# sunshanlu/ORB_SLAM2_ROS2

Hardware: AMD Instinct MI355X
Metric: stereo frames/sec (extract+match) KITTI-00 1241x376; HBM GB/s vs roofline (higher is better)
Workload: dtype u8; 1 GPU; Single 1241x376 KITTI-shaped stereo pair, 8-level pyramid, 2000 FAST+rBRIEF keypoints per image, searchByStereo; batched (512 pairs per step, 512 of them distinct synthetic frames).  `value` is DEVICE-RESIDENT; the checks, rooflines, host_io, sequence job, content sweep, CPU baseline and extra legs run with --full; io=device-resident, n_features=2000, levels=8

## Files before the change

orb_slam2_ros2_amd/csrc/k_brief.hip:

```cpp
#include <hip/hip_runtime.h>
#include <cstdio>
#include <cstring>

#include "orb_math.h"
#include "orbfe_internal.h"
#ifdef BRIEF_STAMPS
namespace orbfe { extern __device__ unsigned long long g_rt_t[4][8]; }
#define RT_STAMP(k) { __syncthreads(); if (tid == 0 && blockIdx.y == 0) orbfe::g_rt_t[k][0] = __builtin_amdgcn_s_memrealtime(); }
#define RTP_STAMP(k) { __syncthreads(); if (tid == 0 && blockIdx.y == 0) orbfe::g_rt_t[k][r] = __builtin_amdgcn_s_memrealtime(); }
#endif
#include "rowtable_body.h"
#include "wave_ops.h"

namespace orbfe {

typedef unsigned long long UmaxPacked;

template <int CTRL, int ROW_MASK>
__device__ __forceinline__ int dpp_i32(int v) {
  return __builtin_amdgcn_update_dpp(0, v, CTRL, ROW_MASK, 0xf, false);
}
__device__ __forceinline__ int wave_sum_i(int v) {
  v += dpp_i32<0x111, 0xf>(v);
  v += dpp_i32<0x112, 0xf>(v);
  v += dpp_i32<0x114, 0xf>(v);
  v += dpp_i32<0x118, 0xf>(v);
  v += dpp_i32<0x142, 0xa>(v);
  v += dpp_i32<0x143, 0xc>(v);
  return __builtin_amdgcn_readlane(v, 63);
}

__device__ __forceinline__ int locate_level(const int32_t* __restrict__ sc, int n_levels, int k, int* j_out, int* total_out) {
  int level = -1, acc = 0, j = 0;
  for (int l = 0; l < n_levels; ++l) {
    const int c = sc[l];
    if (level < 0 && k < acc + c) {
      level = l;
      j = k - acc;
    }
    acc += c;
  }
  *j_out = j;
  *total_out = acc;
  return level;
}

__global__ __launch_bounds__(256) void k_kplist(const LevelDev* __restrict__ lv, int n_levels, const uint32_t* __restrict__ sel,
                                                const int32_t* __restrict__ sel_count, int n_features, uint4* __restrict__ kpl) {
  const int k = blockIdx.x * 256 + threadIdx.x;
  const int img = blockIdx.y;
  if (k >= n_features) return;
  int j, total;
  const int level = locate_level(sel_count + (size_t)img * n_levels, n_levels, k, &j, &total);
  uint4 e = make_uint4(0xFFFFu, 0u, 0u, 0u);
  if (level >= 0) {
    const LevelDev& L = lv[level];
    const uint32_t rec = sel[(size_t)img * n_features + L.quota_off + j];
    e.x = (ORBFE_REC_X(rec) + ORBFE_EDGE) | ((ORBFE_REC_Y(rec) + ORBFE_EDGE) << 16);
    e.y = (uint32_t)level | (ORBFE_REC_R(rec) << 8);
    e.z = L.plane_off;
    e.w = (uint32_t)L.stride;
  }
  kpl[(size_t)img * n_features + k] = e;
}

__global__ __launch_bounds__(256) void k_ic_moments(const uint8_t* __restrict__ pyr, size_t img_pitch, const uint4* __restrict__ kpl,
                                                    int n_features, UmaxPacked umax, int2* __restrict__ moments) {
  __shared__ uint32_t s_mask[256];
  {
    const int it = threadIdx.x >> 4, sb = threadIdx.x & 15;
    const int dy = (sb >> 3) + 2 * it - 15;
    const int ady = dy < 0 ? -dy : dy;
    uint32_t mask = 0u;
    if (ady <= 15) {
      const int d = (int)((umax >> (4 * ady)) & 15ull);
      const int dx0 = 4 * (sb & 7) - 15;
      const int lo = max(0, -d - dx0), hi = min(3, d - dx0);
      mask = (hi >= lo) ? ((0xFFFFFFFFu >> (8 * (3 - hi))) & (0xFFFFFFFFu << (8 * lo))) : 0u;
    }
    s_mask[threadIdx.x] = mask;
  }
  __syncthreads();
  const int lane = threadIdx.x & 63, sub = lane & 15;
  const int k = (blockIdx.x * 4 + (threadIdx.x >> 6)) * 4 + (lane >> 4);
  const int img = blockIdx.y;
  const bool in_range = k < n_features;
  const uint4 e = in_range ? kpl[(size_t)img * n_features + k] : make_uint4(0xFFFFu, 0u, 0u, 0u);
  const bool valid = (e.x & 0xFFFFu) != 0xFFFFu;
  const int x = valid ? (int)(e.x & 0xFFFFu) : 16, y = valid ? (int)(e.x >> 16) : 16;
  const uint8_t* I = pyr + (size_t)img * img_pitch;
  const uint32_t plane = valid ? e.z : 0u;
  const int stride = valid ? (int)e.w : 64;
  constexpr int NIT = 16;
  const uint32_t a0 = plane + (uint32_t)mad24u(y - 15 + (sub >> 3), stride, x - 15 + 4 * (sub & 7));
  const uint32_t step = 2u * (uint32_t)stride;
  uint32_t wv[NIT];
#pragma unroll
  for (int it = 0; it < NIT; ++it) {
    uint32_t w;
    __builtin_memcpy(&w, I + (a0 + (uint32_t)it * step), 4);
    wv[it] = w;
  }
  uint32_t S = 0u, Wp = 0u, T = 0u;
#pragma unroll
  for (int it = 0; it < NIT; ++it) {
    const uint32_t w = wv[it] & s_mask[it * 16 + sub];
    S = __builtin_amdgcn_udot4(w, 0x01010101u, S, false);
    Wp = __builtin_amdgcn_udot4(w, 0x03020100u, Wp, false);
    T = __builtin_amdgcn_udot4(w, 0x01010101u * (uint32_t)it, T, false);
  }
  const int S18 = (int)(S & 0x3FFFFu);
  int m10 = (4 * (sub & 7) - 15) * S18 + (int)Wp;
  int m01 = ((sub >> 3) - 15) * S18 + 2 * (int)T;
#pragma unroll
  for (int sh = 0; sh < 4; ++sh) {
    m10 += (sh == 0) ? dpp_i32<0x111, 0xf>(m10) : (sh == 1) ? dpp_i32<0x112, 0xf>(m10) : (sh == 2) ? dpp_i32<0x114, 0xf>(m10) : dpp_i32<0x118, 0xf>(m10);
    m01 += (sh == 0) ? dpp_i32<0x111, 0xf>(m01) : (sh == 1) ? dpp_i32<0x112, 0xf>(m01) : (sh == 2) ? dpp_i32<0x114, 0xf>(m01) : dpp_i32<0x118, 0xf>(m01);
  }
  if (sub == 15 && valid) moments[(size_t)img * n_features + k] = make_int2(m10, m01);
}

__device__ __forceinline__ KpX kpx_of(const orbfe_keypoint& kp, float sf) {
#pragma clang fp contract(off)
  const float fxq = kp.x / sf, fyq = kp.y / sf;
  int qx = (int)fxq, qy = (int)fyq;
  qx -= (qx > fxq);
  qy -= (qy > fyq);
  KpX r;
  r.x = kp.x;
  r.q = ORBFE_KPX_Q(kp.octave, qx, qy);
  return r;
}

__global__ __launch_bounds__(256) void k_orient(const LevelDev* __restrict__ lv, const uint4* __restrict__ kpl, int n_features,
                                                const int2* __restrict__ moments, double2* __restrict__ sincos,
                                                orbfe_keypoint* __restrict__ kps, KpAux* __restrict__ aux, KpX* __restrict__ kx,
                                                double* __restrict__ theta_out, int rows0, const int32_t* __restrict__ sel_count, int n_levels,
                                                int32_t* __restrict__ n_kp, orbfe_keypoint* __restrict__ kps_host, int32_t* __restrict__ n_kp_host) {
#pragma clang fp contract(off)
  const int k = blockIdx.x * 256 + threadIdx.x;
  const int img = blockIdx.y;
  if (k == 0) {
    int total = 0;
    for (int l = 0; l < n_levels; ++l) total += sel_count[(size_t)img * n_levels + l];
    n_kp[img] = total;
    if (n_kp_host) n_kp_host[img] = total;
  }
  const uint4 e = (k < n_features) ? kpl[(size_t)img * n_features + k] : make_uint4(0xFFFFu, 0u, 0u, 0u);
  if ((e.x & 0xFFFFu) != 0xFFFFu) {
    const int level = (int)(e.y & 0xFFu);
    const LevelDev& L = lv[level];
    const int x = (int)(e.x & 0xFFFFu), y = (int)(e.x >> 16);
    const size_t o = (size_t)img * n_features + k;
    const int2 m = moments[o];
    const double theta = orbmath::det_atan2((double)m.y, (double)m.x);
    double sn, cs;
    orbmath::det_sincos(theta, &sn, &cs);
    sincos[o] = make_double2(sn, cs);
    orbfe_keypoint kp;
    kp.x = (float)x * L.sf;
    kp.y = (float)y * L.sf;
    kp.size = 7.0f;
    kp.angle = (float)(theta / 3.14159265358979323846 * 180);
    kp.response = (float)((e.y >> 8) & 0xFFu);
    kp.octave = level;
    kp.class_id = -1;
    kps[o] = kp;
  #ifndef EXP_NO_KPS_HOST
  if (kps_host) kps_host[o] = kp;
#endif
    kx[o] = kpx_of(kp, L.sf);
    const float r = (float)(2.0 * (double)L.sf);
    const unsigned row = (unsigned)__float2int_rn(kp.y);
    KpAux a;
    a.row_max = (int16_t)min(rows0, __float2int_rn((float)row + r + 1.0f));
    a.row_min = (int16_t)max(0, __float2int_rn((float)row - r));
    aux[o] = a;
    if (theta_out) theta_out[o] = theta;
  }
}

template <bool WITH_ORIENT>
__global__ __launch_bounds__(256) void k_list_moments_orient(const LevelDev* __restrict__ lv, int n_levels, const uint32_t* __restrict__ sel,
                                                             const int32_t* __restrict__ sel_count, int n_features,
                                                             const uint8_t* __restrict__ pyr, size_t img_pitch, UmaxPacked umax,
                                                             uint4* __restrict__ kpl, int2* __restrict__ moments, double2* __restrict__ sincos,
                                                             orbfe_keypoint* __restrict__ kps, KpAux* __restrict__ aux, KpX* __restrict__ kx,
                                                             double* __restrict__ theta_out, int rows0, int32_t* __restrict__ n_kp,
                                                             orbfe_keypoint* __restrict__ kps_host, int32_t* __restrict__ n_kp_host,
                                                             int32_t* __restrict__ rt_flags) {
#pragma clang fp contract(off)
  __shared__ uint32_t s_mask[256];
  if (rt_flags && blockIdx.x == 0 && threadIdx.x < 8) rt_flags[blockIdx.y * 8 + threadIdx.x] = 0;
  {
    const int it = threadIdx.x >> 4, sb = threadIdx.x & 15;
    const int dy = (sb >> 3) + 2 * it - 15;
    const int ady = dy < 0 ? -dy : dy;
    uint32_t mask = 0u;
    if (ady <= 15) {
      const int d = (int)((umax >> (4 * ady)) & 15ull);
      const int dx0 = 4 * (sb & 7) - 15;
      const int lo = max(0, -d - dx0), hi = min(3, d - dx0);
      mask = (hi >= lo) ? ((0xFFFFFFFFu >> (8 * (3 - hi))) & (0xFFFFFFFFu << (8 * lo))) : 0u;
    }
    s_mask[threadIdx.x] = mask;
  }
  __syncthreads();
  const int lane = threadIdx.x & 63, sub = lane & 15;
  const int k = (blockIdx.x * 4 + (threadIdx.x >> 6)) * 4 + (lane >> 4);
  const int img = blockIdx.y;
  const bool in_range = k < n_features;
  uint4 e = make_uint4(0xFFFFu, 0u, 0u, 0u);
  int level = -1, total = 0;
  {
    int j;
    level = locate_level(sel_count + (size_t)img * n_levels, n_levels, in_range ? k : 0x7FFFFFFF, &j, &total);
    if (level >= 0) {
      const LevelDev& L = lv[level];
      const uint32_t rec = sel[(size_t)img * n_features + L.quota_off + j];
      e.x = (ORBFE_REC_X(rec) + ORBFE_EDGE) | ((ORBFE_REC_Y(rec) + ORBFE_EDGE) << 16);
      e.y = (uint32_t)level | (ORBFE_REC_R(rec) << 8);
      e.z = L.plane_off;
      e.w = (uint32_t)L.stride;
    }
  }
  if (WITH_ORIENT && k == 0 && sub == 15) {
    n_kp[img] = total;
    if (n_kp_host) n_kp_host[img] = total;
  }
  const bool valid = (e.x & 0xFFFFu) != 0xFFFFu;
  const int x = valid ? (int)(e.x & 0xFFFFu) : 16, y = valid ? (int)(e.x >> 16) : 16;
  const uint8_t* I = pyr + (size_t)img * img_pitch;
  const uint32_t plane = valid ? e.z : 0u;
  const int stride = valid ? (int)e.w : 64;
  constexpr int NIT = 16;
  const uint32_t a0 = plane + (uint32_t)mad24u(y - 15 + (sub >> 3), stride, x - 15 + 4 * (sub & 7));
  const uint32_t step = 2u * (uint32_t)stride;
  uint32_t wv[NIT];
#pragma unroll
  for (int it = 0; it < NIT; ++it) {
    uint32_t w;
    __builtin_memcpy(&w, I + (a0 + (uint32_t)it * step), 4);
    wv[it] = w;
  }
  uint32_t S = 0u, Wp = 0u, T = 0u;
#pragma unroll
  for (int it = 0; it < NIT; ++it) {
    const uint32_t w = wv[it] & s_mask[it * 16 + sub];
    S = __builtin_amdgcn_udot4(w, 0x01010101u, S, false);
    Wp = __builtin_amdgcn_udot4(w, 0x03020100u, Wp, false);
    T = __builtin_amdgcn_udot4(w, 0x01010101u * (uint32_t)it, T, false);
  }
  const int S18 = (int)(S & 0x3FFFFu);
  int m10 = (4 * (sub & 7) - 15) * S18 + (int)Wp;
  int m01 = ((sub >> 3) - 15) * S18 + 2 * (int)T;
#pragma unroll
  for (int sh = 0; sh < 4; ++sh) {
    m10 += (sh == 0) ? dpp_i32<0x111, 0xf>(m10) : (sh == 1) ? dpp_i32<0x112, 0xf>(m10) : (sh == 2) ? dpp_i32<0x114, 0xf>(m10) : dpp_i32<0x118, 0xf>(m10);
    m01 += (sh == 0) ? dpp_i32<0x111, 0xf>(m01) : (sh == 1) ? dpp_i32<0x112, 0xf>(m01) : (sh == 2) ? dpp_i32<0x114, 0xf>(m01) : dpp_i32<0x118, 0xf>(m01);
  }
  if (sub != 15 || !in_range) return;
  const size_t o = (size_t)img * n_features + k;
  kpl[o] = e;
  if (!valid) return;
  moments[o] = make_int2(m10, m01);
  if (!WITH_ORIENT) return;
  const LevelDev& L = lv[level];
  const double theta = orbmath::det_atan2((double)m01, (double)m10);
  double sn, cs;
  orbmath::det_sincos(theta, &sn, &cs);
  sincos[o] = make_double2(sn, cs);
  orbfe_keypoint kp;
  kp.x = (float)x * L.sf;
  kp.y = (float)y * L.sf;
  kp.size = 7.0f;
  kp.angle = (float)(theta / 3.14159265358979323846 * 180);
  kp.response = (float)((e.y >> 8) & 0xFFu);
  kp.octave = level;
  kp.class_id = -1;
  kps[o] = kp;
#ifndef EXP_NO_KPS_HOST
  if (kps_host) kps_host[o] = kp;
#endif
  kx[o] = kpx_of(kp, L.sf);
  const float r = (float)(2.0 * (double)L.sf);
  const unsigned row = (unsigned)__float2int_rn(kp.y);
  KpAux a;
  a.row_max = (int16_t)min(rows0, __float2int_rn((float)row + r + 1.0f));
  a.row_min = (int16_t)max(0, __float2int_rn((float)row - r));
  aux[o] = a;
  if (theta_out) theta_out[o] = theta;
}

#define BRIEF_R 18
#define BRIEF_ROWS (2 * BRIEF_R + 1)
#define BRIEF_PITCH 48
#define BRIEF_WIN_BYTES 2048

#ifndef BRIEF_WAVES
#define BRIEF_WAVES 4
#endif
#ifndef BRIEF_KPW
#define BRIEF_KPW 2
#endif
#ifdef BRIEF_STAMPS
__device__ unsigned long long g_rt_t[4][8];
__device__ unsigned long long g_bs_rec[8192][6];
#define BS_DECL const unsigned bs_w = ((blockIdx.y * 520u + blockIdx.x) * BRIEF_WAVES + (threadIdx.x >> 6)) & 8191u; const unsigned long long bs_t0 = __builtin_amdgcn_s_memrealtime(); unsigned long long bs_t1 = 0, bs_ta = 0, bs_tb = 0;
#define BS_MID if (!bs_t1) bs_t1 = __builtin_amdgcn_s_memrealtime();
#define BS_END(kind) if ((threadIdx.x & 63) == 0) { asm volatile("s_waitcnt vmcnt(0) lgkmcnt(0)" ::: "memory"); g_bs_rec[bs_w][0] = bs_t0, g_bs_rec[bs_w][1] = bs_t1, g_bs_rec[bs_w][2] = __builtin_amdgcn_s_memrealtime(), g_bs_rec[bs_w][3] = kind, g_bs_rec[bs_w][4] = bs_ta, g_bs_rec[bs_w][5] = bs_tb; }
#else
#define BS_DECL
#define BS_MID
#define BS_END(kind)
#endif
struct BriefRowTable {
  const KpAux* aux;
  const int32_t* n_kp;
  uint32_t* rowoff;
  uint16_t* rowlist;
  int32_t* n_match;
  int rows, list_cap, slot0, n_brief_blocks;
  int stage_cap;
  int32_t* flags;
};
__global__ __launch_bounds__(64 * BRIEF_WAVES) __attribute__((amdgpu_waves_per_eu(8, 8))) void k_brief(const uint8_t* __restrict__ blur, size_t img_pitch,
                                              const uint4* __restrict__ kpl, int n_features, const int8_t* __restrict__ pattern,
                                              const double2* __restrict__ sincos, uint8_t* __restrict__ desc, uint8_t* __restrict__ desc_host,
                                              BriefRowTable rt) {
#pragma clang fp contract(off)
  struct __attribute__((aligned(16))) Lds {
    double rc[BRIEF_WAVES][40];
    uint8_t win[BRIEF_WAVES][2][BRIEF_WIN_BYTES];
    double rs[BRIEF_WAVES][40];
  };
  static_assert(BRIEF_ROWS * BRIEF_PITCH <= BRIEF_WIN_BYTES && BRIEF_WIN_BYTES == 2 * 64 * 16 && BRIEF_PITCH % 16 == 0, "a window is two 16-byte LDS-DMA instructions");
  static_assert((sizeof(double) * 40 * BRIEF_WAVES) % 16 == 0, "the LDS-DMA destination is 16-byte aligned");
  static_assert(sizeof(double) * 40 * BRIEF_WAVES + 2 * BRIEF_WIN_BYTES * BRIEF_WAVES > 255 * 8 &&
                    (sizeof(double) * 40 * BRIEF_WAVES + 2 * BRIEF_WIN_BYTES * BRIEF_WAVES) % 512 != 0,
                "rc[w] and rs[w] must not be reachable by one ds_read2(st64)_b64");
  __shared__ Lds lds;
  BS_DECL
  if (rt.rowoff && (int)blockIdx.x >= rt.n_brief_blocks) {
    static_assert(sizeof(Lds) >= 9000, "the table's row counters borrow the descriptor kernel's LDS (launch_orient_brief checks the row count against 9000 bytes)");
    uint32_t* cnt = (uint32_t*)&lds;
    const int slot = rt.slot0 + (int)blockIdx.y;
    const int r = (int)blockIdx.x - rt.n_brief_blocks;
    if (rt.flags) {
      if (r == 0 && threadIdx.x == 0) rt.n_match[slot >> 1] = 0;
      const int rpw = (rt.rows + 7) >> 3;
      extern __shared__ __attribute__((aligned(16))) uint2 brief_bands[];
      rowtable_build_part(rt.aux + (size_t)blockIdx.y * n_features, min(rt.n_kp[blockIdx.y], n_features), rt.rows, rt.list_cap,
                          rt.rowoff + (size_t)slot * (rt.rows + 1), rt.rowlist + (size_t)slot * rt.list_cap, cnt, cnt + rpw + 12, (int)threadIdx.x, r,
                          rt.flags + (size_t)blockIdx.y * 8, rt.stage_cap > 0 ? brief_bands : nullptr, rt.stage_cap / 4);
      BS_END(2)
      return;
    }
    if (r != 0) return;
    if (threadIdx.x == 0) rt.n_match[slot >> 1] = 0;
    extern __shared__ __attribute__((aligned(16))) uint16_t brief_stage[];
    rowtable_build(rt.aux + (size_t)blockIdx.y * n_features, min(rt.n_kp[blockIdx.y], n_features), rt.rows, rt.list_cap,
                   rt.rowoff + (size_t)slot * (rt.rows + 1), rt.rowlist + (size_t)slot * rt.list_cap, cnt, cnt + rt.rows, (int)threadIdx.x,
                   rt.stage_cap > 0 ? brief_stage : nullptr, rt.stage_cap);
    BS_END(2)
    return;
  }
  const int lane = threadIdx.x & 63;
  const int wave = __builtin_amdgcn_readfirstlane((int)(threadIdx.x >> 6));
  double* rc = lds.rc[wave];
  double* rs = lds.rs[wave];
  const int per_xcd = rt.n_brief_blocks >> 3;
  const int kb = ((int)blockIdx.x & 7) * per_xcd + ((int)blockIdx.x >> 3);
  const int k0 = (kb * BRIEF_WAVES + wave) * BRIEF_KPW;
  const int img = blockIdx.y;
  if (k0 >= n_features) return;
  const uint4* list = kpl + (size_t)img * n_features;
  const double2* sc = sincos + (size_t)img * n_features;
  const uint8_t* W = blur + (size_t)img * img_pitch;
  const int k_last = min(k0 + BRIEF_KPW, n_features) - 1;
  uint32_t tp0 = *(const uint32_t*)(pattern + (0 * 64 + lane) * 4), tp1 = *(const uint32_t*)(pattern + (1 * 64 + lane) * 4);
  uint32_t tp2 = *(const uint32_t*)(pattern + (2 * 64 + lane) * 4), tp3 = *(const uint32_t*)(pattern + (3 * 64 + lane) * 4);
#ifdef BRIEF_STAMPS
  asm volatile("s_waitcnt vmcnt(0)" :: "v"(tp0), "v"(tp1), "v"(tp2), "v"(tp3) : "memory");
  bs_t1 = __builtin_amdgcn_s_memrealtime();
#endif
  const int u1 = min(lane + 64, BRIEF_ROWS * (BRIEF_PITCH / 16) - 1);
  const uint32_t row_a = (uint32_t)lane / 3u, row_b = (uint32_t)u1 / 3u;
  const uint32_t col_a = 16u * ((uint32_t)lane - 3u * row_a), col_b = 16u * ((uint32_t)u1 - 3u * row_b);
  typedef __attribute__((address_space(3))) uint8_t* lds_dst_t;
  typedef const __attribute__((address_space(1))) uint8_t* glb_src_t;
  auto request = [&](const uint4 e, int b) __attribute__((always_inline)) {
    const bool used = (e.x & 0xFFFFu) != 0xFFFFu;
    const int x = used ? (int)(e.x & 0xFFFFu) : BRIEF_R, y = used ? (int)(e.x >> 16) : BRIEF_R;
    const uint32_t plane = used ? e.z : 0u;
    const uint32_t stride = used ? e.w : 0u;
    const uint32_t xa = (uint32_t)(x - BRIEF_R) & ~3u;
    const uint32_t s0 = plane + (uint32_t)(y - BRIEF_R) * stride + xa;
    uint8_t* dst = lds.win[wave][b];
    __builtin_amdgcn_global_load_lds((glb_src_t)(W + (s0 + col_a + __umul24(row_a, stride))), (lds_dst_t)dst, 16, 0, 0);
    __builtin_amdgcn_global_load_lds((glb_src_t)(W + (s0 + col_b + __umul24(row_b, stride))), (lds_dst_t)(dst + 1024), 16, 0, 0);
  };
  uint4 e_cur = list[k0];
  uint4 e_nxt = list[min(k0 + 1, k_last)];
  double2 sc_cur = sc[k0];
#ifdef BRIEF_STAMPS
  asm volatile("s_waitcnt lgkmcnt(0)" ::: "memory");
  bs_ta = __builtin_amdgcn_s_memrealtime();
#endif
  asm volatile("" : "+v"(tp0), "+v"(tp1), "+v"(tp2), "+v"(tp3));
  request(e_cur, 0);
#ifdef BRIEF_STAMPS
  asm volatile("s_waitcnt vmcnt(0)" ::: "memory");
  bs_tb = __builtin_amdgcn_s_memrealtime();
#endif
#pragma unroll
  for (int i = 0; i < BRIEF_KPW; ++i) {
    const int k = k0 + i;
    if (k > k_last) break;
    uint4 e_nn = e_nxt;
    double2 sc_nxt = sc_cur;
    if (i + 2 < BRIEF_KPW) e_nn = list[min(k + 2, k_last)];
    if (i + 1 < BRIEF_KPW && k < k_last) {
      request(e_nxt, (i + 1) & 1);
      sc_nxt = sc[k + 1];
      asm volatile("s_waitcnt vmcnt(2)" ::: "memory");
    } else {
      asm volatile("s_waitcnt vmcnt(0)" ::: "memory");
    }
    __builtin_amdgcn_wave_barrier();
    if ((e_cur.x & 0xFFFFu) != 0xFFFFu) {
      const int x = (int)(e_cur.x & 0xFFFFu), y = (int)(e_cur.x >> 16);
      const int xa = (x - BRIEF_R) & ~3;
      const uint8_t* win = lds.win[wave][i & 1];
      const double sn = sc_cur.x, cs = sc_cur.y;
      if (lane <= 2 * BRIEF_R) {
        const double v = (double)(float)(lane - BRIEF_R);
        rc[lane] = v * cs;
        rs[lane] = v * sn;
      }
      __builtin_amdgcn_fence(__ATOMIC_RELEASE, "wavefront");
      __builtin_amdgcn_wave_barrier();
      BS_MID
      const float px = (float)x, py = (float)y;
      typedef const __attribute__((address_space(3))) uint8_t* lds_bytes_t;
      auto magic_row = [](int y0w) { return (float)(12582912 - (y0w & ~1)); };
      auto magic_col = [](int xa, int y0w, int pitch, int lds_addr) { return (float)(12582912 - xa + lds_addr - (y0w & 1) * pitch); };
      const int y0w = y - BRIEF_R;
      const float magic_y = magic_row(y0w);
      const float magic_x = magic_col(xa, y0w, BRIEF_PITCH, (int)(uint32_t)(uintptr_t)(lds_bytes_t)win);
      auto tests = [&](const uint32_t tpg) __attribute__((always_inline)) -> unsigned long long {
        const int x1 = (int)(int8_t)(tpg & 255u), y1 = (int)(int8_t)((tpg >> 8) & 255u);
        const int x2 = (int)(int8_t)((tpg >> 16) & 255u), y2 = (int)(int8_t)(tpg >> 24);
        const float p1x = (float)(rc[x1 + BRIEF_R] - rs[y1 + BRIEF_R]);
        const float p1y = (float)(rs[x1 + BRIEF_R] + rc[y1 + BRIEF_R]);
        const float p2x = (float)(rc[x2 + BRIEF_R] - rs[y2 + BRIEF_R]);
        const float p2y = (float)(rs[x2 + BRIEF_R] + rc[y2 + BRIEF_R]);
        const uint32_t a1 = (uint32_t)mad24u(__float_as_int((py + p1y) + magic_y), BRIEF_PITCH, __float_as_int((px + p1x) + magic_x)) & 0xFFFFu;
        const uint32_t a2 = (uint32_t)mad24u(__float_as_int((py + p2y) + magic_y), BRIEF_PITCH, __float_as_int((px + p2x) + magic_x)) & 0xFFFFu;
        const int v1 = *(lds_bytes_t)(uintptr_t)a1;
        const int v2 = *(lds_bytes_t)(uintptr_t)a2;
        return __ballot(v1 < v2);
      };
      const unsigned long long bits0 = tests(tp0), bits1 = tests(tp1), bits2 = tests(tp2), bits3 = tests(tp3);
      if (lane < 4) {
        unsigned long long* d64 = (unsigned long long*)(desc + ((size_t)img * n_features + k) * 32);
        unsigned long long b = bits0;
        if (lane == 1) b = bits1;
        if (lane == 2) b = bits2;
        if (lane == 3) b = bits3;
        d64[lane] = b;
        if (desc_host) ((unsigned long long*)(desc_host + ((size_t)img * n_features + k) * 32))[lane] = b;
      }
      __builtin_amdgcn_fence(__ATOMIC_RELEASE, "wavefront");
      __builtin_amdgcn_wave_barrier();
    }
    if (i + 1 < BRIEF_KPW) {
      e_cur = e_nxt;
      e_nxt = e_nn;
      sc_cur = sc_nxt;
    }
  }
  BS_END(1)
}
#ifdef BRIEF_STAMPS
}
extern "C" void orbfe_debug_brief_stamps() {
  static unsigned long long rec[8192][6];
  (void)hipDeviceSynchronize();
  (void)hipMemcpyFromSymbol(rec, HIP_SYMBOL(orbfe::g_bs_rec), sizeof(rec));
  unsigned long long first = ~0ull, last = 0, n = 0, sum = 0, mx = 0, mid = 0, rt0 = 0, rt1 = 0, dlast = 0, sa = 0, sb = 0, ma = 0, mb = 0, smax = 0;
  for (int w = 0; w < 8192; ++w) {
    if (!rec[w][3]) continue;
    first = first < rec[w][0] ? first : rec[w][0], last = last > rec[w][2] ? last : rec[w][2];
    if (rec[w][3] == 1) {
      ++n, sum += rec[w][2] - rec[w][0], mx = mx > rec[w][2] - rec[w][0] ? mx : rec[w][2] - rec[w][0], mid += rec[w][1] ? rec[w][1] - rec[w][0] : 0;
      dlast = dlast > rec[w][2] ? dlast : rec[w][2];
      sa += rec[w][4] - rec[w][0], sb += rec[w][5] - rec[w][4];
      ma = ma > rec[w][4] - rec[w][0] ? ma : rec[w][4] - rec[w][0], mb = mb > rec[w][5] - rec[w][4] ? mb : rec[w][5] - rec[w][4];
    }
  }
  printf("BRIEF stamps (last launch): %llu descriptor waves, launch span %.2f us, last descriptor wave ends at %.2f us; wave mean %.2f max %.2f us, pattern words arrive after %.2f us (mean)\n",
         n, (last - first) * 0.01, (dlast - first) * 0.01, n ? sum * 0.01 / n : 0.0, mx * 0.01, n ? mid * 0.01 / n : 0.0);
  for (int w = 0; w < 8192; ++w)
    if (rec[w][3] == 1) smax = smax > rec[w][0] - first ? smax : rec[w][0] - first;
  printf("  pattern + list entries arrive after %.2f us (mean, max %.2f); window + sin/cos %.2f us later (mean, max %.2f); last descriptor wave starts at %.2f us\n",
         n ? sa * 0.01 / n : 0.0, ma * 0.01, n ? sb * 0.01 / n : 0.0, mb * 0.01, smax * 0.01);
  for (int w = 0; w < 8192; ++w)
    if (rec[w][3] == 2 && (w & 3) == 0) printf("  row-table workgroup: starts %.2f us, ends %.2f us after the launch's first wave\n", (rec[w][0] - first) * 0.01, (rec[w][2] - first) * 0.01);
  {
    unsigned long long rt[4][8];
    (void)hipMemcpyFromSymbol(rt, HIP_SYMBOL(orbfe::g_rt_t), sizeof(rt));
    for (int r = 0; r < 8; ++r)
      printf("  row table part %d (image 0): zeroed %.2f | counted %.2f | lower parts known %.2f | scattered %.2f us after the launch's first wave\n", r,
             (rt[0][r] - first) * 0.01, (rt[1][r] - first) * 0.01, (rt[2][r] - first) * 0.01, (rt[3][r] - first) * 0.01);
  }
  memset(rec, 0, sizeof(rec));
  (void)hipMemcpyToSymbol(HIP_SYMBOL(orbfe::g_bs_rec), rec, sizeof(rec));
  (void)rt0, (void)rt1;
}
namespace orbfe {
#endif

void launch_orient_brief(hipStream_t s, const LevelDev* d_lv, int n_levels, const uint8_t* d_pyr, const uint8_t* d_blur,
                         size_t img_pitch, const uint32_t* d_sel, const int32_t* d_sel_count, int n_features,
                         const int8_t* d_pattern, const int umax[16], orbfe_keypoint* d_kps, uint8_t* d_desc, KpAux* d_aux,
                         int32_t* d_n_kp, double* d_theta, int2* d_moments, double2* d_sincos, KpX* d_kx,
                         uint4* d_kpl, int rows0, int n_img, hipEvent_t before_brief, hipEvent_t before_lists, orbfe_keypoint* h_kps,
                         uint8_t* h_desc, int32_t* h_n_kp, bool fuse_small, uint32_t* d_rowoff_slot, uint16_t* d_rowlist_slot, int32_t* d_n_match,
                         int rt_rows, int rt_list_cap, int rt_slot0, int32_t* d_rt_flags) {
  if (n_img <= 0 || n_features <= 0) return;
  UmaxPacked u = 0;
  for (int i = 0; i < 16; ++i) u |= (unsigned long long)(umax[i] & 15) << (4 * i);
  if (fuse_small && n_img <= 2) {
    if (before_lists) (void)hipStreamWaitEvent(s, before_lists, 0);
    hipLaunchKernelGGL(k_list_moments_orient<true>, dim3((n_features + 15) / 16, n_img), dim3(256), 0, s, d_lv, n_levels, d_sel, d_sel_count, n_features,
                       d_pyr, img_pitch, u, d_kpl, d_moments, d_sincos, d_kps, d_aux, d_kx, d_theta, rows0, d_n_kp, h_kps, h_n_kp,
                       (d_rowoff_slot && d_rt_flags) ? d_rt_flags + (size_t)rt_slot0 * 8 : (int32_t*)nullptr);
    if (before_brief) (void)hipStreamWaitEvent(s, before_brief, 0);
    const int nb = (((n_features + BRIEF_WAVES * BRIEF_KPW - 1) / (BRIEF_WAVES * BRIEF_KPW)) + 7) & ~7;
    BriefRowTable rt{};
    rt.n_brief_blocks = nb;
    if (d_rowoff_slot && (size_t)(rt_rows + 4) * 4 <= 9000)
      rt = BriefRowTable{d_aux, d_n_kp, d_rowoff_slot, d_rowlist_slot, d_n_match, rt_rows, rt_list_cap, rt_slot0, nb, 0,
                         d_rt_flags ? d_rt_flags + (size_t)rt_slot0 * 8 : (int32_t*)nullptr};
    if (rt.rowoff && (rt.flags || rt_list_cap % 8 == 0)) rt.stage_cap = rt.flags ? 4 * std::min(n_features, 4096) : std::min(rt_list_cap, 20480);
    hipLaunchKernelGGL(k_brief, dim3(nb + (rt.rowoff ? 8 : 0), n_img), dim3(64 * BRIEF_WAVES), (size_t)rt.stage_cap * 2, s, d_blur, img_pitch, d_kpl, n_features,
                       d_pattern, d_sincos, d_desc, h_desc, rt);
#ifdef EXP_BRIEF_TWICE
    hipLaunchKernelGGL(k_brief, dim3(nb + (rt.rowoff ? 8 : 0), n_img), dim3(64 * BRIEF_WAVES), 0, s, d_blur, img_pitch, d_kpl, n_features, d_pattern,
                       d_sincos, d_desc, h_desc, rt);
#endif
    return;
  }
  hipLaunchKernelGGL(k_kplist, dim3((n_features + 255) / 256, n_img), dim3(256), 0, s, d_lv, n_levels, d_sel, d_sel_count, n_features,
                     d_kpl);
  hipLaunchKernelGGL(k_ic_moments, dim3((n_features + 15) / 16, n_img), dim3(256), 0, s, d_pyr, img_pitch, d_kpl, n_features, u,
                     d_moments);
  if (before_lists) (void)hipStreamWaitEvent(s, before_lists, 0);
  hipLaunchKernelGGL(k_orient, dim3((n_features + 255) / 256, n_img), dim3(256), 0, s, d_lv, d_kpl, n_features, d_moments, d_sincos,
                     d_kps, d_aux, d_kx, d_theta, rows0, d_sel_count, n_levels, d_n_kp, h_kps, h_n_kp);
  if (before_brief) (void)hipStreamWaitEvent(s, before_brief, 0);
  BriefRowTable rt_none{};
  rt_none.n_brief_blocks = (((n_features + BRIEF_WAVES * BRIEF_KPW - 1) / (BRIEF_WAVES * BRIEF_KPW)) + 7) & ~7;
  hipLaunchKernelGGL(k_brief, dim3(rt_none.n_brief_blocks, n_img), dim3(64 * BRIEF_WAVES), 0, s, d_blur, img_pitch, d_kpl, n_features, d_pattern, d_sincos, d_desc,
                     h_desc, rt_none);
}

}
```

Baseline: 116,600 stereo pairs/s.

## Widen IC-moment loads to 8 bytes and interleave images across blocks

The intensity-centroid moment kernel now has each 16-lane group cover the 31x31 patch as 4 rows by 4 eight-byte column chunks per iteration, using 8 iterations of 8-byte loads instead of 16 iterations of 4-byte loads. The mask table and the dot-product weights are rearranged to match. The grid becomes 1D with blocks interleaved across groups of 8 images, probably to spread concurrent work over memory channels or XCDs. The trade-offs are more index arithmetic and unaligned 8-byte loads, plus some padded blocks when the image count is not a multiple of 8.

Result: no change. 116,400 stereo pairs/s (-0.2%).

```diff
diff --git a/orb_slam2_ros2_amd/csrc/k_brief.hip b/orb_slam2_ros2_amd/csrc/k_brief.hip
--- a/orb_slam2_ros2_amd/csrc/k_brief.hip
+++ b/orb_slam2_ros2_amd/csrc/k_brief.hip
@@ -65,16 +65,16 @@
 }
 
 __global__ __launch_bounds__(256) void k_ic_moments(const uint8_t* __restrict__ pyr, size_t img_pitch, const uint4* __restrict__ kpl,
-                                                    int n_features, UmaxPacked umax, int2* __restrict__ moments) {
-  __shared__ uint32_t s_mask[256];
+                                                    int n_features, UmaxPacked umax, int2* __restrict__ moments, int n_kp_blocks, int n_img) {
+  __shared__ __attribute__((aligned(8))) uint32_t s_mask[256];
   {
-    const int it = threadIdx.x >> 4, sb = threadIdx.x & 15;
-    const int dy = (sb >> 3) + 2 * it - 15;
+    const int j = threadIdx.x & 1, it = threadIdx.x >> 5, sb = (threadIdx.x >> 1) & 15;
+    const int dy = (sb >> 2) + 4 * it - 15;
     const int ady = dy < 0 ? -dy : dy;
     uint32_t mask = 0u;
     if (ady <= 15) {
       const int d = (int)((umax >> (4 * ady)) & 15ull);
-      const int dx0 = 4 * (sb & 7) - 15;
+      const int dx0 = 4 * (2 * (sb & 3) + j) - 15;
       const int lo = max(0, -d - dx0), hi = min(3, d - dx0);
       mask = (hi >= lo) ? ((0xFFFFFFFFu >> (8 * (3 - hi))) & (0xFFFFFFFFu << (8 * lo))) : 0u;
     }
@@ -82,36 +82,43 @@
   }
   __syncthreads();
   const int lane = threadIdx.x & 63, sub = lane & 15;
-  const int k = (blockIdx.x * 4 + (threadIdx.x >> 6)) * 4 + (lane >> 4);
-  const int img = blockIdx.y;
-  const bool in_range = k < n_features;
+  const int per_group = 8 * n_kp_blocks;
+  const int g = (int)blockIdx.x / per_group, L = (int)blockIdx.x - g * per_group;
+  const int img_of_block = 8 * g + (L & 7);
+  const int img = min(img_of_block, n_img - 1);
+  const int k = ((L >> 3) * 4 + (int)(threadIdx.x >> 6)) * 4 + (lane >> 4);
+  const bool in_range = k < n_features && img_of_block < n_img;
   const uint4 e = in_range ? kpl[(size_t)img * n_features + k] : make_uint4(0xFFFFu, 0u, 0u, 0u);
   const bool valid = (e.x & 0xFFFFu) != 0xFFFFu;
   const int x = valid ? (int)(e.x & 0xFFFFu) : 16, y = valid ? (int)(e.x >> 16) : 16;
   const uint8_t* I = pyr + (size_t)img * img_pitch;
   const uint32_t plane = valid ? e.z : 0u;
   const int stride = valid ? (int)e.w : 64;
-  constexpr int NIT = 16;
-  const uint32_t a0 = plane + (uint32_t)mad24u(y - 15 + (sub >> 3), stride, x - 15 + 4 * (sub & 7));
-  const uint32_t step = 2u * (uint32_t)stride;
-  uint32_t wv[NIT];
+  constexpr int NIT = 8;
+  const uint32_t a0 = plane + (uint32_t)mad24u(y - 15 + (sub >> 2), stride, x - 15 + 8 * (sub & 3));
+  const uint32_t step = 4u * (uint32_t)stride;
+  uint2 wv[NIT];
 #pragma unroll
   for (int it = 0; it < NIT; ++it) {
-    uint32_t w;
-    __builtin_memcpy(&w, I + (a0 + (uint32_t)it * step), 4);
+    uint2 w;
+    __builtin_memcpy(&w, I + (a0 + (uint32_t)it * step), 8);
     wv[it] = w;
   }
   uint32_t S = 0u, Wp = 0u, T = 0u;
 #pragma unroll
   for (int it = 0; it < NIT; ++it) {
-    const uint32_t w = wv[it] & s_mask[it * 16 + sub];
-    S = __builtin_amdgcn_udot4(w, 0x01010101u, S, false);
-    Wp = __builtin_amdgcn_udot4(w, 0x03020100u, Wp, false);
-    T = __builtin_amdgcn_udot4(w, 0x01010101u * (uint32_t)it, T, false);
+    const uint2 m = *(const uint2*)&s_mask[(it * 16 + sub) * 2];
+    const uint32_t w0 = wv[it].x & m.x, w1 = wv[it].y & m.y;
+    S = __builtin_amdgcn_udot4(w0, 0x01010101u, S, false);
+    Wp = __builtin_amdgcn_udot4(w0, 0x03020100u, Wp, false);
+    T = __builtin_amdgcn_udot4(w0, 0x01010101u * (uint32_t)it, T, false);
+    S = __builtin_amdgcn_udot4(w1, 0x01010101u, S, false);
+    Wp = __builtin_amdgcn_udot4(w1, 0x07060504u, Wp, false);
+    T = __builtin_amdgcn_udot4(w1, 0x01010101u * (uint32_t)it, T, false);
   }
   const int S18 = (int)(S & 0x3FFFFu);
-  int m10 = (4 * (sub & 7) - 15) * S18 + (int)Wp;
-  int m01 = ((sub >> 3) - 15) * S18 + 2 * (int)T;
+  int m10 = (8 * (sub & 3) - 15) * S18 + (int)Wp;
+  int m01 = ((sub >> 2) - 15) * S18 + 4 * (int)T;
 #pragma unroll
   for (int sh = 0; sh < 4; ++sh) {
     m10 += (sh == 0) ? dpp_i32<0x111, 0xf>(m10) : (sh == 1) ? dpp_i32<0x112, 0xf>(m10) : (sh == 2) ? dpp_i32<0x114, 0xf>(m10) : dpp_i32<0x118, 0xf>(m10);
@@ -554,8 +561,9 @@
   }
   hipLaunchKernelGGL(k_kplist, dim3((n_features + 255) / 256, n_img), dim3(256), 0, s, d_lv, n_levels, d_sel, d_sel_count, n_features,
                      d_kpl);
-  hipLaunchKernelGGL(k_ic_moments, dim3((n_features + 15) / 16, n_img), dim3(256), 0, s, d_pyr, img_pitch, d_kpl, n_features, u,
-                     d_moments);
+  const int n_kp_blocks = (n_features + 15) / 16;
+  hipLaunchKernelGGL(k_ic_moments, dim3((unsigned)((n_img + 7) / 8) * 8u * (unsigned)n_kp_blocks), dim3(256), 0, s, d_pyr, img_pitch, d_kpl,
+                     n_features, u, d_moments, n_kp_blocks, n_img);
   if (before_lists) (void)hipStreamWaitEvent(s, before_lists, 0);
   hipLaunchKernelGGL(k_orient, dim3((n_features + 255) / 256, n_img), dim3(256), 0, s, d_lv, d_kpl, n_features, d_moments, d_sincos,
                      d_kps, d_aux, d_kx, d_theta, rows0, d_sel_count, n_levels, d_n_kp, h_kps, h_n_kp);
```
